# ReadAlongs/SoundSwallower

Hardware: AMD Instinct MI355X
Metric: senone-frames/sec (en-us PTM) (higher is better)
Workload: dtype f32+i32

## Files before the change

### include/ssw_amd.h

```cpp
#ifndef SSW_AMD_H
#define SSW_AMD_H

#include <stddef.h>
#include <stdint.h>

#ifdef __cplusplus
extern "C" {
#endif

#define SSW_ABI_VERSION 2

typedef struct ssw_config_s {
    double logbase;
    double varfloor;
    double mixwfloor;
    double tmatfloor;
    int32_t topn;
    int32_t ds;
    int32_t aw;
    int32_t device;
} ssw_config_t;
#define SSW_DEVICE_NONE (-2)

void ssw_config_defaults(ssw_config_t *cfg);
// ... 32 lines not shown
int ssw_score_batch(ssw_model_t *m, int scorer, const float *d_feats, int32_t n_frames,
                    const int32_t *utt_off, int32_t n_utts, int16_t *d_out, void *stream);
#define SSW_SCORE_CARRY_UTTS 1u
#define SSW_SCORE_SHARE_DEVICE 2u
#define SSW_SCORE_CARRY_OUT_REWIND 4u
int ssw_score_batch_ex(ssw_model_t *m, int scorer, const float *d_feats, int32_t n_frames,
                       const int32_t *utt_off, int32_t n_utts, int16_t *d_out, void *stream,
                       uint32_t flags, const uint32_t *carry_in, uint32_t *carry_out);
int ssw_score_batch_host(ssw_model_t *m, int scorer, const float *feats, int32_t n_frames,
                         const int32_t *utt_off, int32_t n_utts, int16_t *out);
int ssw_score_batch_topn(ssw_model_t *m, int32_t n_frames, uint8_t *cw, int32_t *score);
int ssw_debug_mfma_f16_tiles(ssw_model_t *m, const uint16_t *A, const uint16_t *B, const float *C,
                             float *D, int32_t n_tiles);
int ssw_debug_scan_keys(ssw_model_t *m, const float *d_feats, int32_t n_frames, int32_t cbf,
                        float *keys);
int ssw_score_batch_stats(ssw_model_t *m, int64_t stats[2]);
int ssw_scan_audit_stats(ssw_model_t *m, int64_t stats[2]);

int ssw_set_kernel_timing(ssw_model_t *m, int enable);
int ssw_get_kernel_timing(ssw_model_t *m, float *ms, int n);
int ssw_debug_score_loop(ssw_model_t *m, int scorer, const float *d_feats, int32_t n_frames,
                         const int32_t *utt_off, int32_t n_utts, int16_t *d_out, int32_t reps,
                         void *stream);

typedef struct ssw_mgau_s ssw_mgau_t;
typedef struct ssw_mgaufuncs_s {
    const char *name;
    int (*frame_eval)(ssw_mgau_t *mgau, int16_t *senscr, uint8_t *senone_active,
                      int32_t n_senone_active, float **feat, int32_t frame,
                      int32_t compallsen);
    int (*transform)(ssw_mgau_t *mgau, void *mllr);
    void (*free)(ssw_mgau_t *mgau);
} ssw_mgaufuncs_t;
struct ssw_mgau_s {
    ssw_mgaufuncs_t *vt;
    int frame_idx;
};

ssw_mgau_t *ssw_ptm_mgau_init(ssw_model_t *m);
ssw_mgau_t *ssw_ms_mgau_init(ssw_model_t *m);
void ssw_mgau_reset_hist(ssw_mgau_t *mgau);
int ssw_mgau_prescore(ssw_mgau_t *mgau, const float *feats, int32_t n_frames);

typedef struct ssw_align_entry_s {
    int32_t start, duration, score;
} ssw_align_entry_t;
// ... 291 lines not shown
```

### soundswallower_amd/_lib.py

```python
from __future__ import annotations

import ctypes as C
import os
import subprocess

_HERE = os.path.dirname(os.path.abspath(__file__))
LIB_PATH = os.environ.get("SSW_AMD_LIB") or os.path.join(_HERE, "libssw_amd.so")
CSRC = os.path.join(_HERE, "csrc")
HEADER = os.path.join(os.path.dirname(_HERE), "include", "ssw_amd.h")

_lib = None


class SswConfig(C.Structure):
    _fields_ = [("logbase", C.c_double), ("varfloor", C.c_double), ("mixwfloor", C.c_double),
                ("tmatfloor", C.c_double), ("topn", C.c_int32), ("ds", C.c_int32),
                ("aw", C.c_int32), ("device", C.c_int32)]


class SswModelInfo(C.Structure):
    _fields_ = [(n, C.c_int32) for n in
                ("n_cb", "n_feat", "n_density", "veclen_total", "n_sen", "n_ci_sen", "n_ciphone",
                 "n_phone", "n_emit_state", "n_tmat", "n_sseq", "sil", "n_floored", "topn",
                 "has_ptm", "has_ms", "device")] + [
# ... 65 lines not shown
    L.ssw_model_selftest_message.restype = C.c_char_p
    L.ssw_model_selftest_message.argtypes = [vp]
    L.ssw_model_table.restype = vp
    L.ssw_model_table.argtypes = [vp, C.c_int, C.POINTER(sz)]
    L.ssw_score_batch.argtypes = [vp, C.c_int, vp, i32, vp, i32, vp, vp]
    L.ssw_debug_score_loop.argtypes = [vp, C.c_int, vp, i32, vp, i32, vp, i32, vp]
    L.ssw_score_batch_ex.argtypes = [vp, C.c_int, vp, i32, vp, i32, vp, vp, C.c_uint32, vp, vp]
    L.ssw_score_batch_host.argtypes = [vp, C.c_int, vp, i32, vp, i32, vp]
    L.ssw_score_batch_topn.argtypes = [vp, i32, vp, vp]
    L.ssw_score_batch_stats.argtypes = [vp, vp]
    L.ssw_scan_audit_stats.argtypes = [vp, vp]
    L.ssw_align_stats.argtypes = [vp, vp]
    L.ssw_compact_plan_create.restype = vp
    L.ssw_compact_plan_create.argtypes = [vp, i32, vp, vp, vp, vp]
    L.ssw_compact_plan_free.argtypes = [vp]
    L.ssw_compact_plan_free.restype = None
    L.ssw_compact_plan_elems.argtypes = [vp]
    L.ssw_compact_plan_elems.restype = sz
    L.ssw_compact_plan_rows.argtypes = [vp, i32, vp, vp]
    L.ssw_score_batch_compact.argtypes = [vp, C.c_int, vp, vp, vp, vp, C.c_uint32]
    L.ssw_align_batch_compact.argtypes = [vp, vp, vp, vp, vp, vp, vp, vp, vp, C.c_uint32]
    L.ssw_debug_scan_keys.argtypes = [vp, vp, i32, i32, vp]
    L.ssw_debug_mfma_f16_tiles.argtypes = [vp, vp, vp, vp, vp, i32]
    L.ssw_set_kernel_timing.argtypes = [vp, C.c_int]
    L.ssw_get_kernel_timing.argtypes = [vp, vp, C.c_int]
    L.ssw_ptm_mgau_init.restype = C.POINTER(SswMgau)
    L.ssw_ptm_mgau_init.argtypes = [vp]
    L.ssw_ms_mgau_init.restype = C.POINTER(SswMgau)
    L.ssw_ms_mgau_init.argtypes = [vp]
    L.ssw_mgau_reset_hist.argtypes = [C.POINTER(SswMgau)]
    L.ssw_mgau_prescore.argtypes = [C.POINTER(SswMgau), vp, i32]
    L.ssw_align_batch.argtypes = [vp, vp, i32, vp, vp, vp, vp, vp, vp, vp, vp, vp]
    L.ssw_align_batch_active.argtypes = [vp, vp, i32, vp, vp, vp, vp, vp, vp, vp, vp, vp, vp, vp]
    L.ssw_align_batch_active_ex.argtypes = [vp, C.c_int, vp, i32, vp, vp, vp, vp, vp, vp, vp, vp, vp, vp, vp]
    L.ssw_alignment_propagate.argtypes = [vp, vp, i32, vp, i32]
    L.ssw_state_align_search_init.restype = vp
    L.ssw_state_align_search_init.argtypes = [vp, C.POINTER(SswMgau), i32, vp, vp, vp, vp]
    L.ssw_state_align_search_start.argtypes = [vp]
    L.ssw_state_align_search_step.argtypes = [vp, vp, C.c_int]
    L.ssw_state_align_search_finish.argtypes = [vp]
    L.ssw_state_align_search_n_frames.restype = i32
    L.ssw_state_align_search_n_frames.argtypes = [vp]
    L.ssw_state_align_search_states.restype = C.POINTER(SswAlignEntry)
    L.ssw_state_align_search_states.argtypes = [vp, C.POINTER(i32)]
    L.ssw_state_align_search_phones.restype = C.POINTER(SswAlignEntry)
    L.ssw_state_align_search_phones.argtypes = [vp, C.POINTER(i32)]
# ... 143 lines not shown
```

### soundswallower_amd/api.py

```python
from __future__ import annotations

import ctypes as C
import os

import numpy as np

from . import _lib
from ._lib import SswAlignEntry, SswConfig, SswFeConfig, SswModelInfo

SCORER_PTM = 0
SCORER_MS = 1
SSW_DEVICE_NONE = -2
INT_MAX = 2**31 - 1

_TABLES = {
    "mean": (0, np.float32), "var": (1, np.float32), "det": (2, np.float32),
    "ptm_mixw": (3, np.uint8), "ms_pdf": (4, np.uint8), "tp": (5, np.uint8),
    "sseq": (6, np.uint16), "sen2cb": (7, np.int16), "logadd8": (8, np.uint8),
    "phone_ssid": (9, np.int32), "phone_tmat": (10, np.int32),
    "rec": (11, np.float32), "scan_rec": (12, np.float32), "scan_d0": (13, np.float32),
    "scan_exact": (14, np.uint32), "scan_rec_mfma": (15, np.float32),
    "scan_exact_mfma": (16, np.uint32), "scan_wfrag": (17, np.uint16),
}

# ... 176 lines not shown

    def debug_mfma_f16_tiles(self, A, B, C):
        A = np.ascontiguousarray(A, np.float16)
        B = np.ascontiguousarray(B, np.float16)
        C = np.ascontiguousarray(C, np.float32)
        n = len(A)
        assert A.shape == (n, 32, 16) and B.shape == (n, 16, 32) and C.shape == (n, 32, 32)
        D = np.zeros_like(C)
        _check(self._L.ssw_debug_mfma_f16_tiles(self._m, _ptr(A), _ptr(B), _ptr(C), _ptr(D), n),
               "ssw_debug_mfma_f16_tiles")
        return D

    def debug_scan_keys(self, feats, cbf):
        feats = np.ascontiguousarray(feats, np.float32).reshape(-1, self.veclen_total)
        d = self.to_device(feats)
        out = np.zeros((len(feats), 128), np.float32)
        try:
            _check(self._L.ssw_debug_scan_keys(self._m, d, len(feats), int(cbf), _ptr(out)),
                   "ssw_debug_scan_keys")
        finally:
            self.device_free(d)
        return out

    def set_kernel_timing(self, enable=True):
        _check(self._L.ssw_set_kernel_timing(self._m, int(bool(enable))), "ssw_set_kernel_timing")

    def kernel_timing(self):
        ms = np.zeros(2, np.float32)
        n = _check(self._L.ssw_get_kernel_timing(self._m, _ptr(ms), 2), "ssw_get_kernel_timing")
        self.timing_split = n == 2
        return float(ms[0]), float(ms[1])

    def last_stats(self):
        st = np.zeros(2, np.int64)
        self._L.ssw_score_batch_stats(self._m, _ptr(st))
        return int(st[0]), int(st[1])

    def scan_audit_stats(self):
        st = np.zeros(2, np.int64)
        self._L.ssw_scan_audit_stats(self._m, _ptr(st))
        return int(st[0]), int(st[1])

    def align_stats(self):
        st = np.zeros(2, np.int64)
        self._L.ssw_align_stats(self._m, _ptr(st))
        return int(st[0]), int(st[1])
# ... 948 lines not shown
```

### soundswallower_amd/csrc/ssw_host_active.inc

```

static int
active_first_frames(const int32_t *sf, const int32_t *ef, int n_phones, int n_frames,
                    std::vector<int32_t> &first)
{
    first.assign((size_t)n_phones, INT_MAX);
    int32_t prev_first = 0, prev_last = 0;
    for (int i = 0; i < n_phones; ++i) {
        if (i > 0 && (sf[i] < sf[i - 1] || ef[i] < ef[i - 1])) {
            ssw_set_error("ssw_align_batch_active: phone windows must not decrease along an "
                          "utterance (phone %d); with such windows the reference's active set "
                          "depends on the path scores", i);
            return -1;
        }
        int32_t fi = i == 0 ? 0 : std::max(std::max((int32_t)1, sf[i]), prev_first);
        if (i > 0 && fi > prev_last)
            break;
        if (fi >= n_frames)
            break;
        first[i] = fi;
        prev_first = fi;
        prev_last = ef[i] < fi ? fi : ef[i];
    }
    return 0;
}
// ... 201 lines not shown
                        const uint32_t *seed_active, ssw_align_entry_t *state_io, int32_t *status,
                        int16_t *d_senscr, void *stream, const uint32_t *d_carry_rows)
{
    ModelBusy busy_(m);
    if (!busy_.ok)
        return -1;
    const ssw_host_model_t *h = m->h;
    hipStream_t st = (hipStream_t)stream;
    if (n_utts <= 0)
        return 0;
    if (check_scorer_shape(m, scorer) < 0)
        return -1;
    if (h->n_cb > 64 || h->n_emit_state != 3) {
        ssw_set_error("ssw_align_batch_active: built for <= 64 codebooks and 3-state HMMs");
        return -1;
    }
    if (!d_feats || !frame_off || !phone_off || !senid || !tmatid || !sf || !ef || !state_io
        || !status || frame_off[0] != 0 || phone_off[0] != 0) {
        ssw_set_error("ssw_align_batch_active: bad arguments");
        return -1;
    }
    HIP_OK(hipSetDevice(m->device));
    const int n_frames = frame_off[n_utts];
    std::vector<uint16_t> sen_slot((size_t)h->n_sen, 0);
    {
        std::vector<int> next((size_t)h->n_cb + 1, 0);
        for (int i = 0; i < h->n_sen; ++i)
            ++next[(size_t)h->sen2cb[i] + 1];
        for (int c = 0; c < h->n_cb; ++c)
            next[(size_t)c + 1] = next[(size_t)c] + ((next[(size_t)c + 1] + 3) & ~3);
        for (int i = 0; i < h->n_sen; ++i)
            sen_slot[(size_t)i] = (uint16_t)next[(size_t)h->sen2cb[i]]++;
    }
    std::vector<ActiveUtt> per_utt((size_t)n_utts);
    {
        ActiveJob J;
        J.h = h;
        J.sen_slot = sen_slot.data();
        J.n_utts = n_utts;
        J.frame_off = frame_off;
        J.phone_off = phone_off;
        J.sf = sf;
        J.ef = ef;
        J.senid = senid;
        J.seed_active = seed_active;
        J.out = per_utt.data();
        J.per_chunk = std::max(1, (n_utts + 4 * ssw_host_threads() - 1) / (4 * ssw_host_threads()));
        ssw_parallel_for((n_utts + J.per_chunk - 1) / J.per_chunk, active_build_chunk, &J);
    }
    std::vector<int32_t> seg_of_frame((size_t)std::max(n_frames, 1));
    std::vector<int32_t> seg_utt, seg_nreal, seg_boff(1, 0), utt_real_off((size_t)n_utts + 1, 0);
    std::vector<uint32_t> real_ent, bridge_ent;
    std::vector<uint16_t> real_rank;
    std::vector<unsigned long long> seg_cbmask;
    int cap = 1;
    for (int u = 0; u < n_utts; ++u) {
// ... 102 lines not shown
```

### soundswallower_amd/csrc/ssw_host_model.inc

```

struct Knobs {
    int sen_fpb;
    int sen_r;
    int sen_groups;
    bool sen_generic;
    bool ms_senone_old;
    bool scan_fma;
    int mfma_min_frames;
    int score_piece;
    int host_pipe_cap;
    int mfma_steps;
    bool mfma_balance;
    int mfma_lds_pad;
    bool ptm_exact;
    bool frame_fused;
    int scan_audit;
    float selftest_eps_u;
    bool selftest_off;
    bool align_band, align_win;
    bool align_bt;
    char align_kernel[8];
    int align_band_tokens;
    int align_win_waves;
    bool align_timing;
// ... 96 lines not shown
    ssw_host_model_t *h;
    Knobs kn;
    int scan_mode;
    int selftest_status;
    float selftest_worst_u, selftest_ms;
    char selftest_msg[200];
    int device;
    int n_cu;
    std::atomic<unsigned long long> owner;
    int owner_depth;
    int n_cbf, sen_stride;
    float *d_rec;
    float *d_rec28;
    float *d_recq;
    float *d_recmax;
    uint32_t *d_exlist;
    uint4 *d_wfrag;
    uint32_t *d_exlistm;
    int n_exact_form;
    uint8_t *d_mixw, *d_ms_pdf, *d_sen2cb, *d_logadd8, *d_logadd_mirror, *d_tp, *d_quad_cb;
    short4 *d_slot_sen;
    uint32_t *d_quad_info;
    uint16_t *d_sen_slot;
    unsigned char *d_act_ws;
    size_t act_ws_cap;
    int n_quads, slot_stride;
    uint32_t *d_topn_cw;
    int4 *d_topn_sc;
    int *d_utt_off;
    uint32_t *d_utt_start;
    uint32_t *d_carry0;
    size_t carry_cap;
    uint32_t *d_carry_rows;
    size_t carry_rows_cap;
    unsigned long long *d_nfixed;
    size_t ws_frames, ws_utts, ws_bits, ws_utts_hint, ws_bits_hint, meta_nw;
    std::vector<int32_t> *utt_cache;
    unsigned char *h_stage[2];
    size_t h_stage_cap[2];
    hipEvent_t ev_stage[2];
    int stage_next;
    hipStream_t last_score_stream;
    int have_last_score_stream;
    hipStream_t s_pipe, s_copy;
    hipEvent_t ev_piece[2], ev_down[2];
    unsigned char *h_pipe_feat[2], *h_pipe_out[2];
// ... 176 lines not shown
            T = h->logadd8[i] > T ? h->logadd8[i] : T;
        std::vector<uint8_t> mir((size_t)3 * SSW_LOGADD_MIRROR);
        for (int part = 0; part < 2; ++part) {
            const int size = (part + 1) * SSW_LOGADD_MIRROR, mid = size / 2;
            uint8_t *out = mir.data() + (part ? SSW_LOGADD_MIRROR : 0);
            for (int e = 0; e < size; ++e) {
                const int d = e < mid ? mid - e : e - mid;
                out[e] = (uint8_t)(T - (d < 256 ? (int)h->logadd8[d] : 0));
            }
        }
        HIP_OK(hipMalloc((void **)&m->d_logadd_mirror, mir.size()));
        HIP_OK(hipMemcpy(m->d_logadd_mirror, mir.data(), mir.size(), hipMemcpyHostToDevice));
    }
    if (h->n_sen) {
        std::vector<uint8_t> s2c((size_t)h->n_sen);
        for (int i = 0; i < h->n_sen; ++i)
            s2c[i] = (uint8_t)h->sen2cb[i];
        HIP_OK(hipMalloc((void **)&m->d_sen2cb, s2c.size()));
        HIP_OK(hipMemcpy(m->d_sen2cb, s2c.data(), s2c.size(), hipMemcpyHostToDevice));
    }
    if (h->ptm_mixw || h->ms_pdf) {
        std::vector<int16_t> slot_sen;
        std::vector<uint8_t> quad_cb;
        for (int c = 0; c < h->n_cb; ++c) {
            size_t start = slot_sen.size();
            for (int i = 0; i < h->n_sen; ++i)
                if (h->sen2cb[i] == c)
                    slot_sen.push_back((int16_t)i);
            while ((slot_sen.size() - start) % 4)
                slot_sen.push_back(-1);
            for (size_t q = start / 4; q < slot_sen.size() / 4; ++q)
                quad_cb.push_back((uint8_t)c);
        }
        m->n_quads = (int)quad_cb.size();
        m->slot_stride = ((int)slot_sen.size() + 127) & ~127;
        m->sen_stride = m->slot_stride;
        const size_t rows = (size_t)h->n_feat * h->n_density;
        if (h->ptm_mixw) {
            std::vector<uint8_t> mw(rows * m->slot_stride, 0);
            for (size_t r = 0; r < rows; ++r)
                for (size_t sl = 0; sl < slot_sen.size(); ++sl) {
                    const int sen = slot_sen[sl] >= 0 ? slot_sen[sl] : slot_sen[sl & ~(size_t)3];
                    mw[r * m->slot_stride + sl] = h->ptm_mixw[r * h->n_sen + sen];
                }
            HIP_OK(hipMalloc((void **)&m->d_mixw, mw.size()));
            HIP_OK(hipMemcpy(m->d_mixw, mw.data(), mw.size(), hipMemcpyHostToDevice));
        }
        if (h->ms_pdf) {
            std::vector<uint8_t> mw(rows * m->slot_stride, 0);
            for (size_t sl = 0; sl < slot_sen.size(); ++sl) {
                const int sen = slot_sen[sl] >= 0 ? slot_sen[sl] : slot_sen[sl & ~(size_t)3];
                const uint8_t *src = h->ms_pdf + (size_t)sen * rows;
                for (size_t r = 0; r < rows; ++r)
                    mw[r * m->slot_stride + sl] = src[r];
            }
// ... 3 lines not shown
        {
            std::vector<uint32_t> qi(quad_cb.size());
            for (size_t q = 0; q < qi.size(); ++q) {
                const int16_t *sj = &slot_sen[4 * q];
                const bool run4 = sj[0] >= 0 && sj[1] == sj[0] + 1 && sj[2] == sj[0] + 2
                    && sj[3] == sj[0] + 3;
                qi[q] = ((uint32_t)sj[0] & 0xffffu) | ((uint32_t)run4 << 16)
                    | ((uint32_t)quad_cb[q] << 24);
            }
            HIP_OK(hipMalloc((void **)&m->d_quad_info, qi.size() * sizeof(uint32_t)));
            HIP_OK(hipMemcpy(m->d_quad_info, qi.data(), qi.size() * sizeof(uint32_t),
                             hipMemcpyHostToDevice));
        }
        HIP_OK(hipMalloc((void **)&m->d_quad_cb, quad_cb.size()));
        HIP_OK(hipMemcpy(m->d_quad_cb, quad_cb.data(), quad_cb.size(), hipMemcpyHostToDevice));
        {
            std::vector<uint16_t> sen_slot((size_t)h->n_sen, 0);
            for (size_t sl = 0; sl < slot_sen.size(); ++sl)
                if (slot_sen[sl] >= 0)
                    sen_slot[(size_t)slot_sen[sl]] = (uint16_t)sl;
            HIP_OK(hipMalloc((void **)&m->d_sen_slot, sen_slot.size() * sizeof(uint16_t) + 16));
            HIP_OK(hipMemcpy(m->d_sen_slot, sen_slot.data(), sen_slot.size() * sizeof(uint16_t),
                             hipMemcpyHostToDevice));
        }
        HIP_OK(hipMalloc((void **)&m->d_slot_sen, slot_sen.size() * sizeof(int16_t)));
        HIP_OK(hipMemcpy(m->d_slot_sen, slot_sen.data(), slot_sen.size() * sizeof(int16_t),
                         hipMemcpyHostToDevice));
    }
    if (h->tp) {
        size_t n = (size_t)h->tp_n_tmat * h->tp_n_state * (h->tp_n_state + 1);
        HIP_OK(hipMalloc((void **)&m->d_tp, n + 16));
        HIP_OK(hipMemcpy(m->d_tp, h->tp, n, hipMemcpyHostToDevice));
    }
    return 0;
}

static void
mfma_self_test(ssw_model_s *m)
{
    m->scan_mode = m->d_wfrag != NULL ? 1 : 0;
    m->selftest_status = 0;
    m->selftest_msg[0] = 0;
    if (m->d_wfrag == NULL || m->kn.selftest_off)
        return;
    {
        void *sym = NULL;
// ... 119 lines not shown
    (void)hipFree(m->d_rec);
    (void)hipFree(m->d_rec28);
    (void)hipFree(m->d_recq);
    (void)hipFree(m->d_recmax);
    (void)hipFree(m->d_exlist);
    (void)hipFree(m->d_wfrag);
    (void)hipFree(m->d_exlistm);
    (void)hipFree(m->d_align_ws);
    (void)hipFree(m->d_fp_ws);
    (void)hipFree(m->d_fpa_ws);
    (void)hipFree(m->d_gr_ws);
    (void)hipFree(m->d_text_scr);
    (void)hipFree(m->d_feat_off);
    (void)hipFree(m->d_fe_tab);
    if (m->fe_rate_tab)
        for (auto &kv : *m->fe_rate_tab)
            (void)hipFree(kv.second);
    delete m->fe_rate_tab;
    (void)hipFree(m->d_fe_ws);
    if (m->fe_ev_ready)
        for (int i = 0; i < 4; ++i)
            (void)hipEventDestroy(m->fe_ev[i]);
    (void)hipFree(m->d_sen_slot);
    (void)hipFree(m->d_act_ws);
    (void)hipFree(m->d_mixw);
    (void)hipFree(m->d_ms_pdf);
    (void)hipFree(m->d_sen2cb);
    if (m->s_up) {
        (void)hipEventDestroy(m->ev_up);
        (void)hipStreamDestroy(m->s_up);
    }
    (void)hipFree(m->d_quad_cb);
    (void)hipFree(m->d_quad_info);
    (void)hipFree(m->d_slot_sen);
    (void)hipFree(m->d_logadd8);
    (void)hipFree(m->d_logadd_mirror);
    (void)hipFree(m->d_tp);
    (void)hipFree(m->d_topn_cw);
    (void)hipFree(m->d_topn_sc);
    (void)hipFree(m->d_utt_off);
    (void)hipFree(m->d_carry0);
    (void)hipFree(m->d_carry_rows);
    (void)hipFree(m->d_nfixed);
    delete m->utt_cache;
    delete m->xcd_cuts;
    for (int k = 0; k < 2; ++k) {
// ... 81 lines not shown
    case SSW_TAB_PTM_MIXW: p = h->ptm_mixw; n = (size_t)h->n_feat * h->n_density * h->n_sen; break;
    case SSW_TAB_MS_PDF: p = h->ms_pdf; n = (size_t)h->n_feat * h->n_density * h->n_sen; break;
    case SSW_TAB_TP: p = h->tp; n = (size_t)h->tp_n_tmat * h->tp_n_state * (h->tp_n_state + 1); break;
    case SSW_TAB_SSEQ: p = h->sseq; n = (size_t)h->n_sseq * h->n_emit_state * 2; break;
    case SSW_TAB_SEN2CB: p = h->sen2cb; n = (size_t)h->n_sen * 2; break;
    case SSW_TAB_LOGADD8: p = h->logadd8; n = 256; break;
    case SSW_TAB_PHONE_SSID: p = h->phone_ssid; n = (size_t)h->n_phone * 4; break;
    case SSW_TAB_PHONE_TMAT: p = h->phone_tmat; n = (size_t)h->n_phone * 4; break;
    case SSW_TAB_REC: p = h->rec; n = (size_t)h->n_cb * h->n_feat * h->n_density * SSW_REC_FLOATS * 4; break;
    case SSW_TAB_SCAN_REC: p = h->recq; n = (size_t)h->n_cb * h->n_feat * h->n_density * SSW_REC_FLOATS * 4; break;
    case SSW_TAB_SCAN_D0: p = h->recd0; n = (size_t)h->n_cb * h->n_feat * SSW_REC_FLOATS * 4; break;
    case SSW_TAB_SCAN_EXACT: p = h->exlist; n = (size_t)h->n_cb * h->n_feat * SSW_EXLIST_STRIDE * 4; break;
    case SSW_TAB_SCAN_REC_MFMA: p = h->recqm; n = p ? (size_t)h->n_cb * h->n_feat * h->n_density * SSW_REC_FLOATS * 4 : 0; break;
    case SSW_TAB_SCAN_EXACT_MFMA: p = h->exlistm; n = p ? (size_t)h->n_cb * h->n_feat * SSW_EXLIST_STRIDE * 4 : 0; break;
    case SSW_TAB_SCAN_WFRAG: p = h->wfrag; n = p ? (size_t)h->n_cb * h->n_feat * SSW_WFRAG_PER_CBF * 2 : 0; break;
    default: break;
    }
    if (p == NULL)
        n = 0;
    if (nbytes)
        *nbytes = n;
    return p;
}
```

### soundswallower_amd/csrc/ssw_host_score.inc

```
static int
ensure_score_ws(ssw_model_s *m, int n_frames, int n_utts)
{
    if ((size_t)n_frames > m->ws_frames) {
        (void)hipFree(m->d_topn_cw);
        (void)hipFree(m->d_topn_sc);
        m->d_topn_cw = NULL;
        m->d_topn_sc = NULL;
        m->ws_frames = 0;
        if ((uint64_t)n_frames * (uint64_t)m->n_cbf > 0xffffffffull) {
            ssw_set_error("batch of %d frames is too large (frames x codebooks x streams must fit 32 bits)",
                          n_frames);
            return -1;
        }
        if (dev_alloc(&m->d_topn_cw, (size_t)n_frames * m->n_cbf) < 0
            || dev_alloc(&m->d_topn_sc, (size_t)n_frames * m->n_cbf) < 0)
            return -1;
        m->ws_frames = (size_t)n_frames;
    }
    if (m->d_nfixed == NULL) {
        if (dev_alloc(&m->d_nfixed, 4) < 0)
            return -1;
        HIP_OK(hipMemset(m->d_nfixed, 0, 4 * sizeof(unsigned long long)));
    }
    const size_t need_bits = 2 * (((size_t)n_frames + 31) / 32 + 2);
// ... 102 lines not shown
    S.quad_cb = m->d_quad_cb;
    S.quad_info = m->d_quad_info;
    S.slot_sen = m->d_slot_sen;
    S.logadd8 = m->d_logadd8;
    S.logadd_mirror = m->d_logadd_mirror + (scorer == SSW_SCORER_MS ? SSW_LOGADD_MIRROR : 0);
    S.nfixed = move_stats ? m->d_nfixed : NULL;
    S.nfixed_acc = m->stats_accumulate;
    S.out = d_out;
    if (cp != NULL) {
        S.utt_of_frame = cp->d_utt_of_frame;
        S.cutt_off = cp->d_frame_off;
        S.cstride = cp->d_cstride;
        S.crow_off = cp->d_crow_off;
        S.cpos = cp->d_cpos;
        S.frame_base = frame_base;
    }
    S.n_frames = n_frames;
    S.n_cb = h->n_cb;
    S.n_feat = h->n_feat;
    S.n_density = h->n_density;
    S.n_sen = h->n_sen;
    S.slot_stride = m->slot_stride;
    S.n_quads = m->n_quads;
    S.tab_max = 0;
    for (int i = 0; i < 256; ++i)
        S.tab_max = h->logadd8[i] > S.tab_max ? h->logadd8[i] : S.tab_max;
    if (scorer != SSW_SCORER_MS && 255 + SSW_MAX_NEG_ASCR + 3 * S.tab_max >= SSW_LOGADD_LDS) {
        ssw_set_error("unsupported log-add table (largest entry %d)", S.tab_max);
        return -1;
    }
    const bool ptm = scorer != SSW_SCORER_MS;
    const Knobs &kn = m->kn;
    int fpb = n_frames >= 4 * 512 ? 2 : 1;
    if (kn.sen_fpb != 0 && n_frames >= 4 * 512)
        fpb = kn.sen_fpb;
    size_t lds = 0;
    int R = (m->n_quads + SEN_MAX_THREADS - 1) / SEN_MAX_THREADS;
    const bool ms_packed = !ptm && ms_takes_packed_kernel(m, n_frames);
    if (cp != NULL && !ptm && !ms_packed) {
        ssw_set_error("internal error: compact rows asked of the un-packed ms senone kernel");
        return -1;
    }
    if ((ptm || ms_packed) && fpb == 2 && R < 4) {
        const int r7 = (m->n_quads + 447) / 448;
        R = r7 > R ? (r7 > 4 ? 4 : r7) : R;
    }
// ... 18 lines not shown
        case 1: SSW_MS_LAUNCH(1); break;
        case 2: SSW_MS_LAUNCH(2); break;
        case 3: SSW_MS_LAUNCH(3); break;
        case 4: SSW_MS_LAUNCH(4); break;
        default:
            ssw_set_error("too many senones (%d quads)", m->n_quads);
            return -1;
        }
#undef SSW_MS_LAUNCH
        HIP_OK(hipGetLastError());
        return 0;
    }
    if (threads < fpb * m->n_cbf)
        fpb = 1;
    if (threads < m->n_cbf) {
        ssw_set_error("unsupported senone/codebook shape (%d quads, %d codebook x stream)",
                      m->n_quads, m->n_cbf);
        return -1;
    }
    lds = (ms_packed ? 2 * SSW_LOGADD_MIRROR : SSW_LOGADD_MIRROR)
        + 3 * 4 * (size_t)(ms_packed ? ((h->n_cb + 7) & ~7) : SSW_MAX_FEAT) * fpb + 16 * sizeof(int)
        + 2 * 32 * (size_t)m->n_cbf * fpb
        + 20 * (size_t)((fpb * m->n_cbf + 63) & ~63)
        + 8 * (size_t)R * threads + 16;
    const int n_units = (n_frames + fpb - 1) / fpb;
    int per_cu = 32 / (threads / 64);
    per_cu = per_cu < 1 ? 1 : per_cu;
    int groups = m->n_cu * per_cu;
    if (share_device && groups < (n_units + 7) / 8)
        groups = (n_units + 7) / 8;
    if (kn.sen_groups >= 0)
        groups = kn.sen_groups > 0 ? kn.sen_groups : n_units;
    const dim3 grid(groups < n_units ? groups : n_units);
    const bool nf3 = h->n_feat == 3 && !kn.sen_generic;
    if (fpb != 1 && fpb != 2) {
        ssw_set_error("senone kernel: %d frames per group (1 or 2)", fpb);
        return -1;
    }
#define SSW_SEN_LAUNCH_C(RR, FP, NFV, MSV, CV)                                               \
    hipLaunchKernelGGL((ptm_senone_kernel<4, RR, FP, NFV, MSV, CV>), grid, dim3(threads), lds, st, S)
#define SSW_SEN_LAUNCH_NF(RR, FP, MSV, CV)                                                   \
    if (nf3)                                                                                 \
        SSW_SEN_LAUNCH_C(RR, FP, 3, MSV, CV);                                                \
    else                                                                                     \
        SSW_SEN_LAUNCH_C(RR, FP, 0, MSV, CV)
#define SSW_SEN_LAUNCH_FP(RR, MSV, CV)                                                       \
    if (fpb == 2) {                                                                          \
// ... 828 lines not shown
```

### soundswallower_amd/csrc/ssw_k1b_senone.inc

```

struct SenoneParams {
    const uint32_t *topn_cw;
    const int4 *topn_sc;
    const uint8_t *mixw;
    const uint8_t *quad_cb;
    const short4 *slot_sen;
    const uint32_t *quad_info;
    const uint8_t *logadd8;
    const uint8_t *logadd_mirror;
    unsigned long long *nfixed;
    int16_t *out;
    int n_frames, n_cb, n_feat, n_density, n_sen, slot_stride, n_quads;
    int aw, zero;
    int raw;
    int tab_max;
    const int32_t *utt_of_frame, *cutt_off, *cstride;
    const long long *crow_off;
    const uint32_t *cpos;
    int nfixed_acc;
    int frame_base;
};

constexpr int SEN_MAX_THREADS = 1024;

#define SSW_LOGADD_LDS 512
#define SSW_LOGADD_MIRROR 1024

__device__ __forceinline__ int
fast_logadd(int x, int y, const uint8_t *tab)
{
    const int hi = x > y ? x : y;
    const int r = x < y ? x : y;
    return r - (int)tab[hi - r];
}

typedef unsigned short ushort2v __attribute__((ext_vector_type(2)));
typedef uint32_t uint2u __attribute__((ext_vector_type(2), aligned(2)));

__device__ __forceinline__ uint32_t
pk_min_u16(uint32_t a, uint32_t b)
{
    return __builtin_bit_cast(uint32_t, __builtin_elementwise_min(__builtin_bit_cast(ushort2v, a),
                                                                  __builtin_bit_cast(ushort2v, b)));
// ... 175 lines not shown
#define STL(k)                                                                               \
    if ((threadIdx.x & 63) == 0) {                                                           \
        int wv = blockIdx.x * 11 + (threadIdx.x >> 6);                                       \
        if (wv < 16384)                                                                      \
            g_timeline[wv * 6 + (k)] = __builtin_amdgcn_s_memtime();                        \
    }
#else
#define STL(k)
#endif
    STL(0)
    __builtin_amdgcn_s_setprio(3);
    const int n_feat = NF ? NF : P.n_feat;
    static_assert(TOPN == 4, "top-N block is packed 4 x 8 bit");
    extern __shared__ __align__(16) unsigned char smem[];
    const int n_cbf = P.n_cb * P.n_feat;
    uint8_t *s_tab = smem;
    const int NORM_W = MS ? ((P.n_cb + 7) & ~7) : SSW_MAX_FEAT;
    int *s_norm = reinterpret_cast<int *>(smem + MIRROR);
    int *s_red = s_norm + 3 * NORM_W * FPB;
    uint4 *s_item = reinterpret_cast<uint4 *>(s_red + 16);
    const int n_item_pad = (FPB * n_cbf + 63) & ~63;
    int4 *s_stage_sc = reinterpret_cast<int4 *>(s_item + 2 * 2 * n_cbf * FPB);
    uint32_t *s_stage_cw = reinterpret_cast<uint32_t *>(s_stage_sc + n_item_pad);
    short4 *s_sen4 = reinterpret_cast<short4 *>(s_stage_cw + n_item_pad);

    const int tid = threadIdx.x;
    const int nthr = blockDim.x;
    const uint32_t T = (uint32_t)P.tab_max;
    const int n_units = (P.n_frames + FPB - 1) / FPB;
    const int stride_u = (int)gridDim.x;
    int u = (int)blockIdx.x;
    if (u >= n_units)
        return;

    if ((uint32_t)(uintptr_t)(__attribute__((address_space(3))) unsigned char *)smem != 0u)
        __builtin_trap();

    uint32_t my_a, my_b;
    {
        int fr = 0;
#pragma unroll
        for (int k = 1; k < FPB; ++k)
            fr += tid >= k * n_cbf ? 1 : 0;
        const int i = tid - fr * n_cbf, f = i % n_feat;
        const int nidx = MS ? fr * NORM_W + i / n_feat : fr * SSW_MAX_FEAT + f;
        my_a = (uint32_t)fr | (uint32_t)nidx << 4 | (uint32_t)(f * P.n_density) << 16;
        my_b = (uint32_t)(2 * (i * FPB + fr));
// ... 66 lines not shown
            for (int k = 0; k < TOPN; ++k)
                sp[k] -= e0;
            if (MS) {
                const int a0 = -norm - (int)(3u * T) * n_feat;
                if (a0 < 0 || a0 > 30000)
                    atomicOr(&s_red[12 + ns], 1 << (int)(my_a & 0xfu));
            }
            uint4 *dst = s_item + (2 * buf * n_cbf * FPB + (int)my_b);
            const uint32_t row0 = my_a >> 16;
            dst[0] = make_uint4(__umul24(row0 + (cw0 & 0xffu), (uint32_t)P.slot_stride),
                                __umul24(row0 + ((cw0 >> 8) & 0xffu), (uint32_t)P.slot_stride),
                                __umul24(row0 + ((cw0 >> 16) & 0xffu), (uint32_t)P.slot_stride),
                                __umul24(row0 + (cw0 >> 24), (uint32_t)P.slot_stride));
            reinterpret_cast<uint2 *>(dst + 1)[0]
                = make_uint2(sp[0] | (sp[1] << 16), sp[2] | (sp[3] << 16));
            reinterpret_cast<uint32_t *>(dst + 1)[2] = MS
                ? (uint32_t)((-norm - (int)(3u * T) * n_feat) & 0xffff) * 0x10001u
                : e0 * 0x10001u;
        }
    };

    fetch_item(u);
    uint32_t qi_ld[R];
    short4 sen4_ld[R];
#pragma unroll
    for (int r = 0; r < R; ++r) {
        const int q = r * nthr + tid;
        qi_ld[r] = q < P.n_quads ? P.quad_info[q] : 0u;
        sen4_ld[r] = q < P.n_quads ? P.slot_sen[q] : make_short4(-1, -1, -1, -1);
    }
    constexpr int TAB_DW = MIRROR / 4;
    uint32_t tv[(TAB_DW + 255) / 256] = {};
#pragma unroll
    for (int j = 0; j < (TAB_DW + 255) / 256; ++j) {
        const int e = tid + j * nthr;
        if (e < TAB_DW)
            tv[j] = reinterpret_cast<const uint32_t *>(P.logadd_mirror)[e];
    }
    if (tid < 3 * NORM_W * FPB)
        s_norm[tid] = MS ? 0 : SSW_WORST_SCORE;
    if (3 * NORM_W * FPB > nthr)
        for (int i = tid + nthr; i < 3 * NORM_W * FPB; i += nthr)
            s_norm[i] = MS ? 0 : SSW_WORST_SCORE;
    if (tid < 16)
        s_red[tid] = tid < 12 ? INT_MAX : 0;
    if (P.nfixed != nullptr && blockIdx.x == 0 && tid == 0) {
        P.nfixed[1] = (P.nfixed_acc ? P.nfixed[1] : 0ull) + P.nfixed[0];
        P.nfixed[0] = 0ull;
    }
    lds_barrier();
    norm_item(u, 0);
#pragma unroll
    for (int j = 0; j < (TAB_DW + 255) / 256; ++j)
        if (tid + j * nthr < TAB_DW)
            reinterpret_cast<uint32_t *>(s_tab)[tid + j * nthr] = tv[j];
    lds_barrier();
    stage_item(u, 0, 0);

    const __amdgpu_buffer_rsrc_t mw_rsrc = __builtin_amdgcn_make_buffer_rsrc(
        const_cast<uint8_t *>(P.mixw)
            + (uint32_t)__builtin_amdgcn_readfirstlane((int)((uint32_t)tid & ~63u) * 4),
        (short)4, 64, (int)(1u << 23));
    uint32_t qoff[R];
#pragma unroll
    for (int r = 0; r < R; ++r) {
        const int q = r * nthr + tid;
        const uint32_t qi = qi_ld[r];
        qoff[r] = (qi >> 24) * (uint32_t)(n_feat * FPB * 32) | ((qi >> 16) & 1u);
        s_sen4[q] = sen4_ld[r];
    }

    for (int it = 0;; ++it) {
        const int t0 = u * FPB;
        const int nfr = (P.n_frames - t0) < FPB ? (P.n_frames - t0) : FPB;
        const int u_next = u + stride_u;
        const bool has_next = u_next < n_units;
        const int buf = it & 1, slot = it % 3, slot_next = (it + 1) % 3;
        lds_barrier();
        if (has_next)
            fetch_item_dma(u_next);
        STL(1)
        uint32_t asc2[R][FPB][2];
        const uint4 *item_b = s_item + 2 * buf * n_cbf * FPB;
#pragma unroll
        for (int r = 0; r < R; ++r) {
            const int q = r * nthr + tid;
            const int soff = __builtin_amdgcn_readfirstlane(r * nthr * 4);
#pragma unroll
            for (int fr = 0; fr < FPB; ++fr) {
                const uint32_t dead = (q < P.n_quads && fr < nfr) ? 0u : 0xffffffffu;
                asc2[r][fr][0] = asc2[r][fr][1] = dead;
            }
            if (q < P.n_quads) {
                const uint4 *item_cb = reinterpret_cast<const uint4 *>(
                    reinterpret_cast<const unsigned char *>(item_b) + (qoff[r] & ~1u));
                if (MS) {
#pragma unroll
                    for (int fr = 0; fr < FPB; ++fr)
                        if (fr < nfr)
                            asc2[r][fr][0] = asc2[r][fr][1]
                                = reinterpret_cast<const uint32_t *>(item_cb + 2 * fr + 1)[2];
                }
#pragma unroll
                for (int fr = 0; fr < FPB; ++fr) {
                    {
                        constexpr int NI = R * FPB;
                        const int item = r * FPB + fr;
                        if (item * 4 < NI)
                            __builtin_amdgcn_s_setprio(3);
                        else if (item * 4 < 2 * NI)
                            __builtin_amdgcn_s_setprio(2);
                        else if (item * 4 < 3 * NI)
                            __builtin_amdgcn_s_setprio(1);
                        else
                            __builtin_amdgcn_s_setprio(0);
                    }
                    if (fr < nfr) {
                        if (NF) {
// ... 22 lines not shown
                            const uint4 ro = item_cb[2 * (f * FPB + fr)];
                            const uint4 sc4 = item_cb[2 * (f * FPB + fr) + 1];
                            const uint2 np = make_uint2(sc4.x, sc4.y);
                            if (!MS) {
                                asc2[r][fr][0] += sc4.z;
                                asc2[r][fr][1] += sc4.z;
                            }
                            uint32_t mw[1][TOPN];
                            mw[0][0] = (uint32_t)__builtin_amdgcn_raw_buffer_load_b32(mw_rsrc, (int)ro.x, soff, 0);
                            mw[0][1] = (uint32_t)__builtin_amdgcn_raw_buffer_load_b32(mw_rsrc, (int)ro.y, soff, 0);
                            mw[0][2] = (uint32_t)__builtin_amdgcn_raw_buffer_load_b32(mw_rsrc, (int)ro.z, soff, 0);
                            mw[0][3] = (uint32_t)__builtin_amdgcn_raw_buffer_load_b32(mw_rsrc, (int)ro.w, soff, 0);
                            quad_chains<1, TOPN, MID>(mw, &np, asc2[r][fr]);
                        }
                    }
                }
            }
        }
        STL(2)
        __builtin_amdgcn_s_setprio(3);
        if (has_next)
            take_item_dma(u_next);
        short4 sen4[R];
#pragma unroll
        for (int r = 0; r < R; ++r)
            sen4[r] = s_sen4[r * nthr + tid];
        int c_utt[FPB];
        uint4 c_pos[R][FPB];
        if (COMPACT) {
#pragma unroll
            for (int fr = 0; fr < FPB; ++fr) {
                c_utt[fr] = fr < nfr
                    ? __builtin_amdgcn_readfirstlane(P.utt_of_frame[P.frame_base + t0 + fr]) : 0;
#pragma unroll
                for (int r = 0; r < R; ++r) {
                    const int q = r * nthr + tid;
                    c_pos[r][fr] = (q < P.n_quads && fr < nfr)
                        ? *reinterpret_cast<const uint4 *>(P.cpos + (size_t)c_utt[fr] * P.slot_stride + 4 * q)
                        : make_uint4(0xffffffffu, 0xffffffffu, 0xffffffffu, 0xffffffffu);
                }
            }
        }
#pragma unroll
        for (int fr = 0; fr < FPB; ++fr) {
            uint32_t b2 = 0xffffffffu;
#pragma unroll
            for (int r = 0; r < R; ++r)
                b2 = pk_min_u16(b2, pk_min_u16(asc2[r][fr][0], asc2[r][fr][1]));
            const int lo = (int)(b2 & 0xffffu), hi = (int)(b2 >> 16);
            const int wmin = -wave_max_dpp(-(lo < hi ? lo : hi));
            if ((tid & 63) == 0)
                atomicMin(&s_red[slot * FPB + fr], wmin);
        }
        if (has_next)
            norm_item(u_next, slot_next);
        lds_barrier();
        int best[FPB];
#pragma unroll
        for (int fr = 0; fr < FPB; ++fr)
            best[fr] = s_red[slot * FPB + fr];
        const int marked = MS ? s_red[12 + slot] : 0;
        if (MS && tid == 0)
            s_red[12 + (it + 2) % 3] = 0;
        STL(3)
        if (COMPACT) {
#pragma unroll
            for (int fr = 0; fr < FPB; ++fr) {
                if (fr < nfr) {
                    const int uu = c_utt[fr];
                    const int stride = __builtin_amdgcn_readfirstlane(P.cstride[uu]);
                    const long long ro = P.crow_off[uu]
                        + (long long)(P.frame_base + t0 + fr
                                      - __builtin_amdgcn_readfirstlane(P.cutt_off[uu])) * stride;
                    const uintptr_t rb = reinterpret_cast<uintptr_t>(P.out + ro);
                    const uint32_t rb_lo = (uint32_t)__builtin_amdgcn_readfirstlane((int)(uint32_t)rb);
                    const uint32_t rb_hi = (uint32_t)__builtin_amdgcn_readfirstlane((int)(uint32_t)(rb >> 32));
                    const __amdgpu_buffer_rsrc_t orsrc = __builtin_amdgcn_make_buffer_rsrc(
                        reinterpret_cast<void *>(((uintptr_t)rb_hi << 32) | rb_lo), (short)0,
                        stride * 2, 0x00020000);
                    const uint32_t b2 = (uint32_t)best[fr] * 0x10001u;
#pragma unroll
                    for (int r = 0; r < R; ++r) {
                        const uint32_t lo2 = asc2[r][fr][0] - b2, hi2 = asc2[r][fr][1] - b2;
                        const uint4 cp = c_pos[r][fr];
                        if (cp.x != 0xffffffffu)
                            __builtin_amdgcn_raw_buffer_store_b16((short)(lo2 & 0xffffu), orsrc, (int)cp.x, 0, 0);
                        if (cp.y != 0xffffffffu)
                            asm volatile("buffer_store_short_d16_hi %0, %1, %2, 0 offen"
                                         :: "v"(lo2), "v"(cp.y), "s"(orsrc) : "memory");
                        if (cp.z != 0xffffffffu)
                            __builtin_amdgcn_raw_buffer_store_b16((short)(hi2 & 0xffffu), orsrc, (int)cp.z, 0, 0);
                        if (cp.w != 0xffffffffu)
                            asm volatile("buffer_store_short_d16_hi %0, %1, %2, 0 offen"
                                         :: "v"(hi2), "v"(cp.w), "s"(orsrc) : "memory");
                    }
                }
            }
        } else
#pragma unroll
        for (int r = 0; r < R; ++r) {
            const int q = r * nthr + tid;
            if (q < P.n_quads) {
                const bool run4 = qoff[r] & 1u;
                const int sj[4] = { sen4[r].x, sen4[r].y, sen4[r].z, sen4[r].w };
#pragma unroll
                for (int fr = 0; fr < FPB; ++fr) {
                    if (fr < nfr) {
                        const uint32_t b2 = (uint32_t)best[fr] * 0x10001u;
                        int16_t *orow = P.out + (size_t)(t0 + fr) * P.n_sen;
                        uint2u pk;
                        pk.x = asc2[r][fr][0] - b2;
                        pk.y = asc2[r][fr][1] - b2;
                        if (run4) {
                            *reinterpret_cast<uint2u *>(orow + sj[0]) = pk;
                        } else {
                            const int16_t v[4] = { (int16_t)(pk.x & 0xffffu), (int16_t)(pk.x >> 16),
                                                   (int16_t)(pk.y & 0xffffu), (int16_t)(pk.y >> 16) };
#pragma unroll
                            for (int j = 0; j < 4; ++j)
                                if (sj[j] >= 0)
                                    orow[sj[j]] = v[j];
                        }
                    }
                }
            }
        }
        STL(4)
        if (MS && marked != 0) {
            for (int fr = 0; fr < nfr; ++fr)
                if ((marked >> fr) & 1)
                    ms_exact_frame<R, COMPACT>(P, t0 + fr, tid, nthr, reinterpret_cast<int *>(s_stage_cw));
        }
        if (!has_next)
            break;
        stage_item(u_next, slot_next, buf ^ 1);
        if (tid < NORM_W * FPB)
            s_norm[slot * NORM_W * FPB + tid] = MS ? 0 : SSW_WORST_SCORE;
        if (tid < FPB)
            s_red[slot_next * FPB + tid] = INT_MAX;
        u = u_next;
    }
#undef STL
}

// ... 479 lines not shown
```

Before: 64.15 million.

## Reorder senone quads so contiguous runs come first and store via encoded offsets

The quad layout is reordered at model load so every quad holding four consecutive senones comes first, and the index of the first irregular quad is recorded. In the senone kernel, regular wavefronts store each frame's quad with a single dwordx2 store using a senone offset packed into qoff. This drops the per-thread slot_sen staging in LDS and its reload, and only irregular wavefronts read slot_sen from global memory. The best-score broadcast is also hoisted into a scalar-packed form, and the host reuses a cached sen_slot table. The cost is a more complex layout invariant, and the packed offset assumes senone indices fit in the upper bits of qoff.

```diff
diff --git a/include/ssw_amd.h b/include/ssw_amd.h
--- a/include/ssw_amd.h
+++ b/include/ssw_amd.h
@@ -78,6 +78,7 @@
 int ssw_debug_score_loop(ssw_model_t *m, int scorer, const float *d_feats, int32_t n_frames,
                          const int32_t *utt_off, int32_t n_utts, int16_t *d_out, int32_t reps,
                          void *stream);
+int ssw_debug_senone_layout(ssw_model_t *m, int16_t *slot_sen, uint32_t *quad_info, int32_t info[3]);
 
 typedef struct ssw_mgau_s ssw_mgau_t;
 typedef struct ssw_mgaufuncs_s {
diff --git a/soundswallower_amd/_lib.py b/soundswallower_amd/_lib.py
--- a/soundswallower_amd/_lib.py
+++ b/soundswallower_amd/_lib.py
@@ -111,6 +111,8 @@
     L.ssw_align_batch_compact.argtypes = [vp, vp, vp, vp, vp, vp, vp, vp, vp, C.c_uint32]
     L.ssw_debug_scan_keys.argtypes = [vp, vp, i32, i32, vp]
     L.ssw_debug_mfma_f16_tiles.argtypes = [vp, vp, vp, vp, vp, i32]
+    if hasattr(L, "ssw_debug_senone_layout"):
+        L.ssw_debug_senone_layout.argtypes = [vp, vp, vp, vp]
     L.ssw_set_kernel_timing.argtypes = [vp, C.c_int]
     L.ssw_get_kernel_timing.argtypes = [vp, vp, C.c_int]
     L.ssw_ptm_mgau_init.restype = C.POINTER(SswMgau)
diff --git a/soundswallower_amd/api.py b/soundswallower_amd/api.py
--- a/soundswallower_amd/api.py
+++ b/soundswallower_amd/api.py
@@ -222,6 +222,16 @@
             self.device_free(d)
         return out
 
+    def debug_senone_layout(self):
+        info = np.zeros(3, np.int32)
+        _check(self._L.ssw_debug_senone_layout(self._m, None, None, _ptr(info)),
+               "ssw_debug_senone_layout")
+        slot_sen = np.zeros((int(info[0]), 4), np.int16)
+        quad_info = np.zeros(int(info[0]), np.uint32)
+        _check(self._L.ssw_debug_senone_layout(self._m, _ptr(slot_sen), _ptr(quad_info), _ptr(info)),
+               "ssw_debug_senone_layout")
+        return slot_sen, quad_info, int(info[1])
+
     def set_kernel_timing(self, enable=True):
         _check(self._L.ssw_set_kernel_timing(self._m, int(bool(enable))), "ssw_set_kernel_timing")
 
diff --git a/soundswallower_amd/csrc/ssw_host_active.inc b/soundswallower_amd/csrc/ssw_host_active.inc
--- a/soundswallower_amd/csrc/ssw_host_active.inc
+++ b/soundswallower_amd/csrc/ssw_host_active.inc
@@ -247,16 +247,11 @@
     }
     HIP_OK(hipSetDevice(m->device));
     const int n_frames = frame_off[n_utts];
-    std::vector<uint16_t> sen_slot((size_t)h->n_sen, 0);
-    {
-        std::vector<int> next((size_t)h->n_cb + 1, 0);
-        for (int i = 0; i < h->n_sen; ++i)
-            ++next[(size_t)h->sen2cb[i] + 1];
-        for (int c = 0; c < h->n_cb; ++c)
-            next[(size_t)c + 1] = next[(size_t)c] + ((next[(size_t)c + 1] + 3) & ~3);
-        for (int i = 0; i < h->n_sen; ++i)
-            sen_slot[(size_t)i] = (uint16_t)next[(size_t)h->sen2cb[i]]++;
-    }
+    if (m->h_sen_slot == NULL) {
+        ssw_set_error("ssw_align_batch_active: the model has no mixture weights");
+        return -1;
+    }
+    const std::vector<uint16_t> &sen_slot = *m->h_sen_slot;
     std::vector<ActiveUtt> per_utt((size_t)n_utts);
     {
         ActiveJob J;
diff --git a/soundswallower_amd/csrc/ssw_host_model.inc b/soundswallower_amd/csrc/ssw_host_model.inc
--- a/soundswallower_amd/csrc/ssw_host_model.inc
+++ b/soundswallower_amd/csrc/ssw_host_model.inc
@@ -142,6 +142,8 @@
     short4 *d_slot_sen;
     uint32_t *d_quad_info;
     uint16_t *d_sen_slot;
+    std::vector<uint16_t> *h_sen_slot;
+    int first_irregular_quad;
     unsigned char *d_act_ws;
     size_t act_ws_cap;
     int n_quads, slot_stride;
@@ -364,15 +366,32 @@
     if (h->ptm_mixw || h->ms_pdf) {
         std::vector<int16_t> slot_sen;
         std::vector<uint8_t> quad_cb;
-        for (int c = 0; c < h->n_cb; ++c) {
-            size_t start = slot_sen.size();
-            for (int i = 0; i < h->n_sen; ++i)
-                if (h->sen2cb[i] == c)
-                    slot_sen.push_back((int16_t)i);
-            while ((slot_sen.size() - start) % 4)
-                slot_sen.push_back(-1);
-            for (size_t q = start / 4; q < slot_sen.size() / 4; ++q)
-                quad_cb.push_back((uint8_t)c);
+        {
+            std::vector<int16_t> grouped;
+            std::vector<uint8_t> grouped_cb;
+            for (int c = 0; c < h->n_cb; ++c) {
+                size_t start = grouped.size();
+                for (int i = 0; i < h->n_sen; ++i)
+                    if (h->sen2cb[i] == c)
+                        grouped.push_back((int16_t)i);
+                while ((grouped.size() - start) % 4)
+                    grouped.push_back(-1);
+                for (size_t q = start / 4; q < grouped.size() / 4; ++q)
+                    grouped_cb.push_back((uint8_t)c);
+            }
+            for (int pass = 0; pass < 2; ++pass) {
+                if (pass == 1)
+                    m->first_irregular_quad = (int)quad_cb.size();
+                for (size_t q = 0; q < grouped_cb.size(); ++q) {
+                    const int16_t *sj = &grouped[4 * q];
+                    const bool run4 = sj[0] >= 0 && sj[1] == sj[0] + 1 && sj[2] == sj[0] + 2
+                        && sj[3] == sj[0] + 3;
+                    if (run4 == (pass == 0)) {
+                        slot_sen.insert(slot_sen.end(), sj, sj + 4);
+                        quad_cb.push_back(grouped_cb[q]);
+                    }
+                }
+            }
         }
         m->n_quads = (int)quad_cb.size();
         m->slot_stride = ((int)slot_sen.size() + 127) & ~127;
@@ -422,6 +441,7 @@
             HIP_OK(hipMalloc((void **)&m->d_sen_slot, sen_slot.size() * sizeof(uint16_t) + 16));
             HIP_OK(hipMemcpy(m->d_sen_slot, sen_slot.data(), sen_slot.size() * sizeof(uint16_t),
                              hipMemcpyHostToDevice));
+            m->h_sen_slot = new std::vector<uint16_t>(sen_slot);
         }
         HIP_OK(hipMalloc((void **)&m->d_slot_sen, slot_sen.size() * sizeof(int16_t)));
         HIP_OK(hipMemcpy(m->d_slot_sen, slot_sen.data(), slot_sen.size() * sizeof(int16_t),
@@ -587,6 +607,7 @@
         for (int i = 0; i < 4; ++i)
             (void)hipEventDestroy(m->fe_ev[i]);
     (void)hipFree(m->d_sen_slot);
+    delete m->h_sen_slot;
     (void)hipFree(m->d_act_ws);
     (void)hipFree(m->d_mixw);
     (void)hipFree(m->d_ms_pdf);
@@ -714,3 +735,23 @@
         *nbytes = n;
     return p;
 }
+
+extern "C" int
+ssw_debug_senone_layout(ssw_model_t *m, int16_t *slot_sen, uint32_t *quad_info, int32_t info[3])
+{
+    if (m == NULL || m->device == SSW_DEVICE_NONE || m->d_slot_sen == NULL || info == NULL) {
+        ssw_set_error("ssw_debug_senone_layout: no device tables");
+        return -1;
+    }
+    HIP_OK(hipSetDevice(m->device));
+    info[0] = m->n_quads;
+    info[1] = m->first_irregular_quad;
+    info[2] = m->slot_stride;
+    if (slot_sen != NULL)
+        HIP_OK(hipMemcpy(slot_sen, m->d_slot_sen, (size_t)m->n_quads * 4 * sizeof(int16_t),
+                         hipMemcpyDeviceToHost));
+    if (quad_info != NULL)
+        HIP_OK(hipMemcpy(quad_info, m->d_quad_info, (size_t)m->n_quads * sizeof(uint32_t),
+                         hipMemcpyDeviceToHost));
+    return 0;
+}
diff --git a/soundswallower_amd/csrc/ssw_host_score.inc b/soundswallower_amd/csrc/ssw_host_score.inc
--- a/soundswallower_amd/csrc/ssw_host_score.inc
+++ b/soundswallower_amd/csrc/ssw_host_score.inc
@@ -148,6 +148,7 @@
     S.n_sen = h->n_sen;
     S.slot_stride = m->slot_stride;
     S.n_quads = m->n_quads;
+    S.first_irregular_quad = m->first_irregular_quad;
     S.tab_max = 0;
     for (int i = 0; i < 256; ++i)
         S.tab_max = h->logadd8[i] > S.tab_max ? h->logadd8[i] : S.tab_max;
@@ -212,7 +213,12 @@
         + 3 * 4 * (size_t)(ms_packed ? ((h->n_cb + 7) & ~7) : SSW_MAX_FEAT) * fpb + 16 * sizeof(int)
         + 2 * 32 * (size_t)m->n_cbf * fpb
         + 20 * (size_t)((fpb * m->n_cbf + 63) & ~63)
-        + 8 * (size_t)R * threads + 16;
+        + 16;
+    if (32 * (size_t)m->n_cbf * fpb > 65536) {
+        ssw_set_error("unsupported senone/codebook shape (%d quads, %d codebook x stream)",
+                      m->n_quads, m->n_cbf);
+        return -1;
+    }
     const int n_units = (n_frames + fpb - 1) / fpb;
     int per_cu = 32 / (threads / 64);
     per_cu = per_cu < 1 ? 1 : per_cu;
diff --git a/soundswallower_amd/csrc/ssw_k1b_senone.inc b/soundswallower_amd/csrc/ssw_k1b_senone.inc
--- a/soundswallower_amd/csrc/ssw_k1b_senone.inc
+++ b/soundswallower_amd/csrc/ssw_k1b_senone.inc
@@ -19,6 +19,7 @@
     const uint32_t *cpos;
     int nfixed_acc;
     int frame_base;
+    int first_irregular_quad;
 };
 
 constexpr int SEN_MAX_THREADS = 1024;
@@ -240,7 +241,6 @@
     const int n_item_pad = (FPB * n_cbf + 63) & ~63;
     int4 *s_stage_sc = reinterpret_cast<int4 *>(s_item + 2 * 2 * n_cbf * FPB);
     uint32_t *s_stage_cw = reinterpret_cast<uint32_t *>(s_stage_sc + n_item_pad);
-    short4 *s_sen4 = reinterpret_cast<short4 *>(s_stage_cw + n_item_pad);
 
     const int tid = threadIdx.x;
     const int nthr = blockDim.x;
@@ -353,12 +353,10 @@
 
     fetch_item(u);
     uint32_t qi_ld[R];
-    short4 sen4_ld[R];
 #pragma unroll
     for (int r = 0; r < R; ++r) {
         const int q = r * nthr + tid;
         qi_ld[r] = q < P.n_quads ? P.quad_info[q] : 0u;
-        sen4_ld[r] = q < P.n_quads ? P.slot_sen[q] : make_short4(-1, -1, -1, -1);
     }
     constexpr int TAB_DW = MIRROR / 4;
     uint32_t tv[(TAB_DW + 255) / 256] = {};
@@ -395,11 +393,14 @@
     uint32_t qoff[R];
 #pragma unroll
     for (int r = 0; r < R; ++r) {
-        const int q = r * nthr + tid;
         const uint32_t qi = qi_ld[r];
-        qoff[r] = (qi >> 24) * (uint32_t)(n_feat * FPB * 32) | ((qi >> 16) & 1u);
-        s_sen4[q] = sen4_ld[r];
-    }
+        qoff[r] = (qi >> 24) * (uint32_t)(n_feat * FPB * 32) | ((qi >> 16) & 1u) | (qi << 17);
+    }
+    bool irregular[R];
+#pragma unroll
+    for (int r = 0; r < R; ++r)
+        irregular[r] = __builtin_amdgcn_readfirstlane(r * nthr + (tid & ~63)) + 64
+            > P.first_irregular_quad;
 
     for (int it = 0;; ++it) {
         const int t0 = u * FPB;
@@ -410,6 +411,9 @@
         lds_barrier();
         if (has_next)
             fetch_item_dma(u_next);
+#pragma unroll
+        for (int r = 0; r < R; ++r)
+            asm volatile("" : "+v"(qoff[r]));
         STL(1)
         uint32_t asc2[R][FPB][2];
         const uint4 *item_b = s_item + 2 * buf * n_cbf * FPB;
@@ -424,7 +428,7 @@
             }
             if (q < P.n_quads) {
                 const uint4 *item_cb = reinterpret_cast<const uint4 *>(
-                    reinterpret_cast<const unsigned char *>(item_b) + (qoff[r] & ~1u));
+                    reinterpret_cast<const unsigned char *>(item_b) + (qoff[r] & 0xfffeu));
                 if (MS) {
 #pragma unroll
                     for (int fr = 0; fr < FPB; ++fr)
@@ -493,9 +497,19 @@
         if (has_next)
             take_item_dma(u_next);
         short4 sen4[R];
-#pragma unroll
-        for (int r = 0; r < R; ++r)
-            sen4[r] = s_sen4[r * nthr + tid];
+        if (!COMPACT) {
+#pragma unroll
+            for (int r = 0; r < R; ++r) {
+                const int q = r * nthr + tid;
+                if (irregular[r] && q < P.n_quads) {
+                    uint32_t lane_q = (uint32_t)tid;
+                    asm volatile("" : "+v"(lane_q));
+                    sen4[r] = *reinterpret_cast<const short4 *>(
+                        reinterpret_cast<const unsigned char *>(P.slot_sen)
+                        + (lane_q + (uint32_t)(r * nthr)) * 8u);
+                }
+            }
+        }
         int c_utt[FPB];
         uint4 c_pos[R][FPB];
         if (COMPACT) {
@@ -526,10 +540,12 @@
         if (has_next)
             norm_item(u_next, slot_next);
         lds_barrier();
-        int best[FPB];
-#pragma unroll
-        for (int fr = 0; fr < FPB; ++fr)
-            best[fr] = s_red[slot * FPB + fr];
+        uint32_t best2[FPB];
+#pragma unroll
+        for (int fr = 0; fr < FPB; ++fr) {
+            const uint32_t b = (uint32_t)__builtin_amdgcn_readfirstlane(s_red[slot * FPB + fr]);
+            best2[fr] = b | (b << 16);
+        }
         const int marked = MS ? s_red[12 + slot] : 0;
         if (MS && tid == 0)
             s_red[12 + (it + 2) % 3] = 0;
@@ -549,7 +565,7 @@
                     const __amdgpu_buffer_rsrc_t orsrc = __builtin_amdgcn_make_buffer_rsrc(
                         reinterpret_cast<void *>(((uintptr_t)rb_hi << 32) | rb_lo), (short)0,
                         stride * 2, 0x00020000);
-                    const uint32_t b2 = (uint32_t)best[fr] * 0x10001u;
+                    const uint32_t b2 = best2[fr];
 #pragma unroll
                     for (int r = 0; r < R; ++r) {
                         const uint32_t lo2 = asc2[r][fr][0] - b2, hi2 = asc2[r][fr][1] - b2;
@@ -572,25 +588,39 @@
         for (int r = 0; r < R; ++r) {
             const int q = r * nthr + tid;
             if (q < P.n_quads) {
-                const bool run4 = qoff[r] & 1u;
-                const int sj[4] = { sen4[r].x, sen4[r].y, sen4[r].z, sen4[r].w };
-#pragma unroll
-                for (int fr = 0; fr < FPB; ++fr) {
-                    if (fr < nfr) {
-                        const uint32_t b2 = (uint32_t)best[fr] * 0x10001u;
-                        int16_t *orow = P.out + (size_t)(t0 + fr) * P.n_sen;
-                        uint2u pk;
-                        pk.x = asc2[r][fr][0] - b2;
-                        pk.y = asc2[r][fr][1] - b2;
-                        if (run4) {
-                            *reinterpret_cast<uint2u *>(orow + sj[0]) = pk;
-                        } else {
-                            const int16_t v[4] = { (int16_t)(pk.x & 0xffffu), (int16_t)(pk.x >> 16),
-                                                   (int16_t)(pk.y & 0xffffu), (int16_t)(pk.y >> 16) };
-#pragma unroll
-                            for (int j = 0; j < 4; ++j)
-                                if (sj[j] >= 0)
-                                    orow[sj[j]] = v[j];
+                if (!irregular[r]) {
+                    const uint32_t voff = qoff[r] >> 16;
+#pragma unroll
+                    for (int fr = 0; fr < FPB; ++fr) {
+                        if (fr < nfr) {
+                            const int16_t *orow = P.out + (size_t)(t0 + fr) * P.n_sen;
+                            const unsigned long long pk
+                                = (unsigned long long)(asc2[r][fr][0] - best2[fr])
+                                | (unsigned long long)(asc2[r][fr][1] - best2[fr]) << 32;
+                            asm volatile("global_store_dwordx2 %0, %1, %2"
+                                         :: "v"(voff), "v"(pk), "s"(orow) : "memory");
+                        }
+                    }
+                } else {
+                    const bool run4 = qoff[r] & 1u;
+                    const int sj[4] = { sen4[r].x, sen4[r].y, sen4[r].z, sen4[r].w };
+#pragma unroll
+                    for (int fr = 0; fr < FPB; ++fr) {
+                        if (fr < nfr) {
+                            int16_t *orow = P.out + (size_t)(t0 + fr) * P.n_sen;
+                            uint2u pk;
+                            pk.x = asc2[r][fr][0] - best2[fr];
+                            pk.y = asc2[r][fr][1] - best2[fr];
+                            if (run4) {
+                                *reinterpret_cast<uint2u *>(orow + sj[0]) = pk;
+                            } else {
+                                const int16_t v[4] = { (int16_t)(pk.x & 0xffffu), (int16_t)(pk.x >> 16),
+                                                       (int16_t)(pk.y & 0xffffu), (int16_t)(pk.y >> 16) };
+#pragma unroll
+                                for (int j = 0; j < 4; ++j)
+                                    if (sj[j] >= 0)
+                                        orow[sj[j]] = v[j];
+                            }
                         }
                     }
                 }
```

Result: no change. 64.36 million (median of 6 runs) (+0.3%).
